# jmg049/Spectrograms

Hardware: AMD Instinct MI355X
Metric: STFT frames/sec (f32, n_fft=1024 hop=256) (higher is better)
Workload: dtype f32

## Files before the change

spectrograms_amd/csrc/kernels_r32x16.hip:

```cpp
#include <type_traits>
#include <utility>

#include "binaural_kind.h"
#include "buffer_ops.h"
#include "fft_inreg.h"
#include "r32x16_layout.h"
#include "sgx_internal.h"

namespace sgx {
namespace {

using namespace inreg;
using namespace r32x16;

typedef int v4i __attribute__((ext_vector_type(4)));
typedef int v2i __attribute__((ext_vector_type(2)));

__device__ __forceinline__ float db_f32(float x) { return __builtin_log2f(x) * 3.01029995663981195f; }

template <int AMP>
__device__ __forceinline__ float amp_f32(float p, float eps) {
    if constexpr (AMP == AMP_MAGNITUDE) return sqrtf(p);
    else if constexpr (AMP == AMP_DB) return db_f32(fmaxf(p, eps));
    else return p;
}
__device__ __forceinline__ float power_of(v2f x) { return __builtin_fmaf(x.x, x.x, x.y * x.y); }

__device__ __forceinline__ unsigned lds_addr(const void *p) { return (unsigned)(size_t)p; }

#ifdef SGX_STAMPS
__device__ unsigned long long g_stamps[32];
#define SGX_STAMP(i)                                                                        \
    do {                                                                                    \
        unsigned long long t_;                                                              \
        __builtin_amdgcn_sched_barrier(0);                                                  \
        asm volatile("s_memtime %0\n\ts_waitcnt lgkmcnt(0)" : "=s"(t_)::"memory");          \
        __builtin_amdgcn_sched_barrier(0);                                                  \
        st_acc[i] += t_ - st_prev;                                                          \
        st_prev = t_;                                                                       \
    } while (0)
#define SGX_STAMP_PARAMS , unsigned long long *st_acc, unsigned long long &st_prev
#define SGX_STAMP_ARGS , st_acc, st_prev
#else
#define SGX_STAMP(i)
#define SGX_STAMP_PARAMS
#define SGX_STAMP_ARGS
#endif

#ifndef SGX_BANDSEG
#define SGX_BANDSEG 0
#endif
#ifndef SGX_BANDTRIP
#define SGX_BANDTRIP 0
#endif
#ifndef SGX_BANDFMA
#define SGX_BANDFMA 0
#endif
#ifndef SGX_BANDPF
#define SGX_BANDPF 0
#endif
#ifndef SGX_ODDHOP
#define SGX_ODDHOP 1
#endif
#ifndef SGX_DMA
#define SGX_DMA 0
#endif
#ifndef SGX_ONEPATH
#define SGX_ONEPATH 1
#endif

template <int OFF>
__device__ __forceinline__ void ds_read64(v2f &d, unsigned addr) {
    asm volatile("ds_read_b64 %0, %1 offset:%2" : "=v"(d) : "v"(addr), "n"(OFF));
}
template <int OFF>
__device__ __forceinline__ void ds_read128(v4f &d, unsigned addr) {
    asm volatile("ds_read_b128 %0, %1 offset:%2" : "=v"(d) : "v"(addr), "n"(OFF));
}
template <int N>
__device__ __forceinline__ void tie8(v2f *d) {
    if constexpr (N >= 0)
        asm volatile("s_waitcnt lgkmcnt(%8)"
                     : "+v"(d[0]), "+v"(d[1]), "+v"(d[2]), "+v"(d[3]), "+v"(d[4]), "+v"(d[5]), "+v"(d[6]), "+v"(d[7])
                     : "n"(N));
    else
        asm volatile("" : "+v"(d[0]), "+v"(d[1]), "+v"(d[2]), "+v"(d[3]), "+v"(d[4]), "+v"(d[5]), "+v"(d[6]), "+v"(d[7]));
}
template <int N>
__device__ __forceinline__ void tie16(v2f (&d)[16]) {
    tie8<N>(&d[0]);
    tie8<-1>(&d[8]);
}
template <bool XSPAD, int N1>
constexpr int col_off() { return N1 * 128 + (XSPAD ? (N1 >> 3) * 128 : 0); }
template <bool XSPAD, int PAR, int... K>
__device__ __forceinline__ void read_cols(v2f (&x)[16], v2f (&w)[16], unsigned xaddr, unsigned waddr, std::integer_sequence<int, K...>) {
    ((ds_read64<col_off<XSPAD, 2 * K + PAR>()>(x[K], xaddr), ds_read64<(2 * K + PAR) * 128>(w[K], waddr)), ...);
}

template <int HOP>
constexpr int p512_off_a(int n1) { return 64 * n1 + (64 * n1 / (8 * HOP)) * 64; }
template <int HOP>
constexpr int p512_off_b(int n1) { return 64 * n1 + 4 * HOP + ((64 * n1 + 4 * HOP) / (8 * HOP)) * 64; }
template <int O0, int O1>
__device__ __forceinline__ void ds_read2x32(v2f &d, unsigned addr) {
    static_assert(O0 >= 0 && O0 < 256 && O1 >= 0 && O1 < 256, "ds_read2_b32: 8-bit dword offsets");
    asm volatile("ds_read2_b32 %0, %1 offset0:%2 offset1:%3" : "=v"(d) : "v"(addr), "n"(O0), "n"(O1));
}
template <int HOP, int PAR, int... K>
__device__ __forceinline__ void read_cols512(v2f (&x)[16], v2f (&w)[16], const unsigned (&base)[8], unsigned waddr, std::integer_sequence<int, K...>) {
    ((ds_read2x32<(p512_off_a<HOP>(2 * K + PAR) - p512_off_a<HOP>((2 * K + PAR) & ~3)) / 4, (p512_off_b<HOP>(2 * K + PAR) - p512_off_a<HOP>((2 * K + PAR) & ~3)) / 4>(
          x[K], base[(2 * K + PAR) >> 2]),
      ds_read64<(2 * K + PAR) * 128>(w[K], waddr)),
     ...);
}

template <int PAR, int... K>
__device__ __forceinline__ void read_cols_odd(v2f (&x)[16], v2f (&w)[16], const unsigned (&base)[4], unsigned waddr, std::integer_sequence<int, K...>) {
    ((ds_read2x32<((2 * K + PAR) & 7) * 32, ((2 * K + PAR) & 7) * 32 + 1>(x[K], base[(2 * K + PAR) >> 3]), ds_read64<(2 * K + PAR) * 128>(w[K], waddr)), ...);
}

template <int PAR, int... K>
__device__ __forceinline__ void read_win(v2f (&w)[16], unsigned waddr, std::integer_sequence<int, K...>) {
    (ds_read64<(2 * K + PAR) * 128>(w[K], waddr), ...);
}

template <int OFF>
__device__ __forceinline__ void dma16_to_lds(__amdgpu_buffer_rsrc_t r, int voff, unsigned lds_base) {
    unsigned keep;
    asm volatile("s_mov_b32 %0, m0\n\ts_mov_b32 m0, %3\n\ts_nop 0\n\tbuffer_load_dwordx4 %1, %2, 0 offen offset:%4 lds\n\ts_mov_b32 m0, %0"
                 : "=&s"(keep)
                 : "v"(voff), "s"(r), "s"(lds_base), "n"(OFF)
                 : "memory");
}
template <bool XSPAD, int R, int ROUNDS>
__device__ __forceinline__ void dma_rounds(__amdgpu_buffer_rsrc_t r, int voff, unsigned xs_base, unsigned wave) {
    if constexpr (R < ROUNDS) {
        const unsigned c0 = R * 256u + wave * 64u;
        dma16_to_lds<0>(r, voff + R * 4096, xs_base + c0 * 16u + (XSPAD ? (c0 >> 6) * 128u : 0u));
        dma_rounds<XSPAD, R + 1, ROUNDS>(r, voff, xs_base, wave);
    }
}

template <bool CONJ>
__device__ __forceinline__ v2f cmul_reg(v2f x, v2f t) {
    const v2f c = x * lo2(t);
    v2f r;
    if constexpr (CONJ) asm("v_pk_fma_f32 %0, %1, %2, %3 op_sel:[1,1,0] op_sel_hi:[0,1,1] neg_hi:[0,1,0]" : "=v"(r) : "v"(x), "v"(t), "v"(c));
    else asm("v_pk_fma_f32 %0, %1, %2, %3 op_sel:[1,1,0] op_sel_hi:[0,1,1] neg_lo:[0,1,0]" : "=v"(r) : "v"(x), "v"(t), "v"(c));
    return r;
}
__device__ __forceinline__ v2f split_tw(v2f D, v2f w) {
    const v2f c = lo2(D) * w;
    v2f r;
    asm("v_pk_fma_f32 %0, %1, %2, %3 op_sel:[1,1,0] op_sel_hi:[1,0,1] neg_lo:[0,1,0]" : "=v"(r) : "v"(D), "v"(w), "v"(c));
    return r;
}

__device__ __forceinline__ void load_tw1(const StftArgs &a, unsigned n2, v2f (&twa)[4], v2f (&twb)[8]) {
    const v2f *t1 = (const v2f *)a.tw1 + n2;
#pragma unroll
    for (int q = 0; q < 4; ++q) twa[q] = t1[16 * 8 * q];
#pragma unroll
    for (int q = 0; q < 8; ++q) twb[q] = t1[16 * q];
}

template <bool P2>
__device__ __forceinline__ void twiddle_store(v2f (&xr)[32], const v2f (&twa)[4], const v2f (&twb)[8], unsigned char *dst) {
#pragma unroll
    for (int k1 = 0; k1 < 32; ++k1) {
        const int qa = k1 >> 3, qb = k1 & 7;
        v2f r = xr[k1];
        if constexpr (P2) {
            if (k1 == 0) r = cmul_reg<true>(r, twa[2]);
        } else {
            if (qb) r = cmulv(r, twb[qb]);
            if (qa) r = cmulv(r, twa[qa]);
        }
#if defined(SGX_ABL_NOEXW)
        asm volatile("" ::"v"(r), "v"(dst));
#elif defined(SGX_ABL_ADDTID)
        asm volatile("ds_write_addtid_b32 %0 offset:%2\n\tds_write_addtid_b32 %1 offset:%3" ::"v"(r.x), "v"(r.y), "n"(k1 * 512), "n"(k1 * 512 + 256) : "memory");
#else
        *(v2f *)(dst + k1 * 128) = r;
#endif
    }
}

__device__ __forceinline__ void read_rows(const unsigned char *exf, unsigned ra, unsigned rb, v2f (&A)[16], v2f (&B)[16]) {
    const v4f *pa = (const v4f *)(exf + ra * 128);
    const v4f *pb = (const v4f *)(exf + rb * 128);
#pragma unroll
    for (int c = 0; c < 8; ++c) {
        const v4f q = pa[c];
        A[2 * c] = (v2f){q.x, q.y};
        A[2 * c + 1] = (v2f){q.z, q.w};
    }
#pragma unroll
    for (int c = 0; c < 8; ++c) {
        const v4f q = pb[c];
        B[2 * c] = (v2f){q.x, q.y};
        B[2 * c + 1] = (v2f){q.z, q.w};
    }
}

struct JobOfs {
    unsigned a1, b1, a2, b2, mid;
};
__device__ __forceinline__ JobOfs job_offsets(unsigned j, unsigned n_frames) {
    const unsigned c1 = j == 0 ? 16u : j, c2 = j == 0 ? 0u : j + 256u;
    return JobOfs{c1 * n_frames, (512u - 224u - c1) * n_frames, c2 * n_frames, (512u - 224u - c2) * n_frames, 256u * n_frames};
}

__device__ __forceinline__ void pass2_twiddle(v2f (&A)[16], v2f (&B)[16], const v2f (&t)[16]) {
#pragma unroll
    for (int n = 1; n < 16; ++n) {
        A[n] = cmul_reg<false>(A[n], t[n]);
        B[n] = cmul_reg<true>(B[n], t[n]);
    }
}

struct PwAddr {
    float *up, *down;
};
template <int MODE, int AMP, bool PWT, bool ROT>
__device__ __forceinline__ void pass2_compute(v2f (&A)[16], v2f (&B)[16], bool j0, float eps, const v4f *tw, __amdgpu_buffer_rsrc_t ro,
                                              unsigned oa1, unsigned ob1, unsigned oa2, unsigned ob2, unsigned omid, unsigned step,
                                              float *pw_c1, float *pw_m1, float *pw_c2, float *pw_m2, float *pw_mid SGX_STAMP_PARAMS) {
    constexpr int R = ROT ? 1 : 0;
    Fft<16, false>::run(A, A);
    Fft<16, false>::run(B, B);
    const v2f a8 = ROT ? B[9] : A[8];
    if (j0) {
        if constexpr (ROT) {
            v2f nA[8], nB[16];
#pragma unroll
            for (int t = 0; t < 8; ++t) nA[t] = B[t + 1];
#pragma unroll
            for (int i = 0; i < 8; ++i) nB[(16 - i) & 15] = A[15 - i];
#pragma unroll
            for (int t = 0; t < 8; ++t) nB[8 - t] = B[(17 - t) & 15];
#pragma unroll
            for (int t = 0; t < 8; ++t) A[8 + t] = nA[t];
#pragma unroll
            for (int i = 0; i < 16; ++i) B[i] = nB[i];
        } else {
            v2f nA[16], nB[8];
#pragma unroll
            for (int i = 0; i < 8; ++i) { nA[i] = B[i]; nA[8 + i] = A[i]; }
            nB[7] = A[0];
#pragma unroll
            for (int t = 1; t < 8; ++t) nB[7 - t] = A[16 - t];
#pragma unroll
            for (int i = 0; i < 16; ++i) A[i] = nA[i];
#pragma unroll
            for (int i = 0; i < 8; ++i) B[i] = nB[i];
        }
        asm volatile("" ::: "memory");
    }
    SGX_STAMP(9);
    constexpr int PSTEP = MODE == OUT_BINAURAL ? 32 * 16 * 2 : PWT ? 32 * 16 : 32;
    auto emit = [&](unsigned voff, unsigned soff, float *pwp, v2f X, bool conj) {
#ifdef SGX_ABL_NOSTORE
        asm volatile("" ::"v"(X), "v"(voff));
        return;
#endif
        if constexpr (MODE == OUT_COMPLEX) {
            const v2f V = conj ? (v2f){X.x, -X.y} : X;
            __builtin_amdgcn_raw_buffer_store_b64(__builtin_bit_cast(v2i, V), ro, (int)voff, (int)soff, 0);
        } else if constexpr (MODE == OUT_MEL) {
#ifdef SGX_ABL_NOPW
            asm volatile("" ::"v"(X), "v"(pwp));
            return;
#endif
            *pwp = AMP == AMP_MAG_IN ? sqrtf(power_of(X)) : power_of(X);
        } else if constexpr (MODE == OUT_BINAURAL) {
            *(v2f *)pwp = conj ? (v2f){X.x, -X.y} : X;
        } else {
            __builtin_amdgcn_raw_buffer_store_b32(__builtin_bit_cast(int, amp_f32<AMP>(power_of(X), eps)), ro, (int)voff, (int)soff, 0);
        }
    };
    auto twi = [&](int i) {
        const v4f q = tw[i >> 1];
        return (i & 1) ? (v2f){q.z, q.w} : (v2f){q.x, q.y};
    };
    auto split = [&](v2f P, v2f Q, v2f w, v2f &X, v2f &Y) {
        const v2f E = pfma(Q, (v2f){1.f, -1.f}, P);
        const v2f D = pfma(Q, (v2f){-1.f, 1.f}, P);
        const v2f T = split_tw(D, w);
        X = E + T;
        Y = E - T;
    };
#pragma unroll
    for (int i = 0; i < 8; ++i) {
        v2f X, Y;
        split(A[i], B[(15 + R - i) & 15], twi(i), X, Y);
        emit(oa1, i * step, pw_c1 + i * PSTEP, X, false);
        emit(ob1, (7 - i) * step, pw_m1 + (7 - i) * PSTEP, Y, true);
    }
#pragma unroll
    for (int t = 0; t < 8; ++t) {
        v2f X, Y;
        split(A[8 + t], B[7 + R - t], twi(8 + t), X, Y);
        emit(oa2, t * step, pw_c2 + t * PSTEP, X, false);
        emit(ob2, (7 - t) * step, pw_m2 + (7 - t) * PSTEP, Y, true);
    }
    if (j0) emit(omid, 0u, pw_mid, a8 * (v2f){2.f, -2.f}, false);
    SGX_STAMP(10);
}

constexpr unsigned kP512Step = 16u * 64u;
template <int MODE, int AMP, bool PACK = false>
__device__ __forceinline__ void pass2_pair512(v2f (&A)[16], v2f (&B)[16], bool j0, float eps, __amdgpu_buffer_rsrc_t ro, unsigned vfull1,
                                              unsigned vhalf1, unsigned vfull2, unsigned vhalf2, unsigned vfullm, unsigned vhalfm, unsigned step,
                                              float *pw1, float *pw2, float *pwm) {
    Fft<16, false>::run(A, A);
    Fft<16, false>::run(B, B);
    const v2f a8 = A[8];
    if (j0) {
        v2f nA[16], nB[8];
#pragma unroll
        for (int i = 0; i < 8; ++i) { nA[i] = B[i]; nA[8 + i] = A[i]; }
        nB[7] = A[0];
#pragma unroll
        for (int t = 1; t < 8; ++t) nB[7 - t] = A[16 - t];
#pragma unroll
        for (int i = 0; i < 16; ++i) A[i] = nA[i];
#pragma unroll
        for (int i = 0; i < 8; ++i) B[i] = nB[i];
        asm volatile("" ::: "memory");
    }
    auto emit = [&](unsigned vfull, unsigned vhalf, int soff, v2f Xa, v2f Xb, bool conj, float *pwp) {
        if constexpr (MODE == OUT_MEL) {
            const float pa = power_of(Xa), pb = power_of(Xb);
            *(v2f *)pwp = AMP == AMP_MAG_IN ? (v2f){sqrtf(pa), sqrtf(pb)} : (v2f){pa, pb};
        } else if constexpr (MODE == OUT_COMPLEX) {
            const float sg = conj ? -1.f : 1.f;
            const v4f V = (v4f){Xa.x, sg * Xa.y, Xb.x, sg * Xb.y};
            if constexpr (PACK) {
                __builtin_amdgcn_raw_buffer_store_b64(__builtin_bit_cast(v2i, (v2f){V.x, V.y}), ro, (int)vfull, soff, 0);
                __builtin_amdgcn_raw_buffer_store_b64(__builtin_bit_cast(v2i, (v2f){V.z, V.w}), ro, (int)vhalf, soff, 0);
            } else {
                __builtin_amdgcn_raw_buffer_store_b128(__builtin_bit_cast(v4i, V), ro, (int)vfull + soff, 0, 0);
                __builtin_amdgcn_raw_buffer_store_b64(__builtin_bit_cast(v2i, (v2f){V.x, V.y}), ro, (int)vhalf, soff, 0);
            }
        } else {
            const v2f V = (v2f){amp_f32<AMP>(power_of(Xa), eps), amp_f32<AMP>(power_of(Xb), eps)};
            if constexpr (PACK) {
                const float va = V.x, vb = V.y;
                __builtin_amdgcn_raw_buffer_store_b32(__builtin_bit_cast(int, va), ro, (int)vfull, soff, 0);
                __builtin_amdgcn_raw_buffer_store_b32(__builtin_bit_cast(int, vb), ro, (int)vhalf, soff, 0);
            } else {
                __builtin_amdgcn_raw_buffer_store_b64(__builtin_bit_cast(v2i, V), ro, (int)vfull, soff, 0);
                __builtin_amdgcn_raw_buffer_store_b32(__builtin_bit_cast(int, V.x), ro, (int)vhalf, soff, 0);
            }
        }
// ... 273 lines not shown
    const unsigned n = lane & 15u, q = lane >> 4;
    const bool mine = mt < a.mfcc_mtiles;
    v4acc acc = {0.f, 0.f, 0.f, 0.f};
    if (mine) {
        const v4f *pa = (const v4f *)(frag + ((size_t)mt * 64u + lane) * RL);
        const v4f *pb = (const v4f *)(mq + (q * 16u + n) * RL);
        v4f wa[STEPS / 4], vb[STEPS / 4];
#pragma unroll
        for (int g = 0; g < STEPS / 4; ++g) { wa[g] = pa[g]; vb[g] = pb[g]; }
#pragma unroll
        for (int g = 0; g < STEPS / 4; ++g) {
            acc = __builtin_amdgcn_mfma_f32_16x16x4f32(wa[g].x, vb[g].x, acc, 0, 0, 0);
            acc = __builtin_amdgcn_mfma_f32_16x16x4f32(wa[g].y, vb[g].y, acc, 0, 0, 0);
            acc = __builtin_amdgcn_mfma_f32_16x16x4f32(wa[g].z, vb[g].z, acc, 0, 0, 0);
            acc = __builtin_amdgcn_mfma_f32_16x16x4f32(wa[g].w, vb[g].w, acc, 0, 0, 0);
        }
    }
    const float *lift = frag + (size_t)a.mfcc_mtiles * 64u * RL;
    constexpr unsigned kDrop = 0x80000000u;
    const unsigned rows = a.n_mfcc - a.mfcc_skip;
    const unsigned obytes = (rows * a.n_frames - f0) * 4u;
    const __amdgpu_buffer_rsrc_t ro = make_rsrc((const float *)a.out + (size_t)b * rows * a.n_frames + f0, obytes);
    const unsigned mtr = mine ? mt : 0u;
#pragma unroll
    for (int r = 0; r < 4; ++r) {
        const unsigned c = 16u * mtr + 4u * q + r;
        const bool ok = mine && c >= a.mfcc_skip && c < a.n_mfcc && n < nf;
        __builtin_amdgcn_raw_buffer_store_b32(__builtin_bit_cast(int, acc[r] * lift[min(c, a.n_mfcc - 1u)]), ro,
                                              (int)(ok ? ((c - a.mfcc_skip) * a.n_frames + n) * 4u : kDrop), 0, 0);
    }
}

__host__ __device__ constexpr unsigned pwt512_index(unsigned k, unsigned f) { return (k >> 1) * 64u + (f >> 1) * 4u + (k & 1u) * 2u + (f & 1u); }
template <int AMP>
__device__ __forceinline__ void mel_tile_sched512(const StftArgs &a, const float *pwT, const unsigned *sched, unsigned b, unsigned f0,
                                                  unsigned nf, float eps, unsigned tid) {
    const unsigned wave = __builtin_amdgcn_readfirstlane(tid >> 6), lane = tid & 63u, slot = lane >> 4, fp = lane & 15u;
    const unsigned obytes = (a.n_out * a.n_frames - f0) * 4u;
    const __amdgpu_buffer_rsrc_t ro = make_rsrc((const float *)a.out + (size_t)b * a.n_out * a.n_frames + f0, obytes);
    constexpr unsigned kDrop = 0x80000000u;
    const unsigned fo0 = 2u * fp < nf ? 8u * fp : kDrop, fo1 = 2u * fp + 1u < nf ? 8u * fp + 4u : kDrop;
    const uint4 *info = (const uint4 *)(sched + kSchedHdr) + wave * 8u + slot;
    uint4 ca = info[0], cb = info[4];
#pragma unroll
    for (unsigned seg = 0; seg < (unsigned)kSchedSegs; ++seg) {
        const uint4 na = info[(seg + 1u) * 32u], nb = info[(seg + 1u) * 32u + 4u];
        const unsigned L = __builtin_amdgcn_readfirstlane(ca.x);
        const v4f *wa = (const v4f *)((const float *)sched + ca.y), *wb = (const v4f *)((const float *)sched + cb.y);
        const v4f *pa = (const v4f *)(pwT + (ca.z >> 1) * 64u) + fp, *pb = (const v4f *)(pwT + (cb.z >> 1) * 64u) + fp;
        v2f acca = {0.0f, 0.0f}, accb = {0.0f, 0.0f};
        for (unsigned t = 0; t < L; t += 4u) {
            const v4f w4a = wa[t >> 2], a0 = pa[(t >> 1) * 16u], a1 = pa[(t >> 1) * 16u + 16u];
            const v4f w4b = wb[t >> 2], b0 = pb[(t >> 1) * 16u], b1 = pb[(t >> 1) * 16u + 16u];
            acca = mul_add_unfused(w4a.x, (v2f){a0.x, a0.y}, acca);
            accb = mul_add_unfused(w4b.x, (v2f){b0.x, b0.y}, accb);
            acca = mul_add_unfused(w4a.y, (v2f){a0.z, a0.w}, acca);
            accb = mul_add_unfused(w4b.y, (v2f){b0.z, b0.w}, accb);
            acca = mul_add_unfused(w4a.z, (v2f){a1.x, a1.y}, acca);
            accb = mul_add_unfused(w4b.z, (v2f){b1.x, b1.y}, accb);
            acca = mul_add_unfused(w4a.w, (v2f){a1.z, a1.w}, acca);
            accb = mul_add_unfused(w4b.w, (v2f){b1.z, b1.w}, accb);
        }
        const bool ha = ca.w != 0xffffffffu, hb = cb.w != 0xffffffffu;
        const unsigned boa = ca.w * a.n_frames * 4u, bob = cb.w * a.n_frames * 4u;
        __builtin_amdgcn_raw_buffer_store_b32(__builtin_bit_cast(int, amp_f32<AMP>(acca.x, eps)), ro, (int)((ha && fo0 != kDrop) ? boa + fo0 : kDrop), 0, 0);
        __builtin_amdgcn_raw_buffer_store_b32(__builtin_bit_cast(int, amp_f32<AMP>(acca.y, eps)), ro, (int)((ha && fo1 != kDrop) ? boa + fo1 : kDrop), 0, 0);
        __builtin_amdgcn_raw_buffer_store_b32(__builtin_bit_cast(int, amp_f32<AMP>(accb.x, eps)), ro, (int)((hb && fo0 != kDrop) ? bob + fo0 : kDrop), 0, 0);
        __builtin_amdgcn_raw_buffer_store_b32(__builtin_bit_cast(int, amp_f32<AMP>(accb.y, eps)), ro, (int)((hb && fo1 != kDrop) ? bob + fo1 : kDrop), 0, 0);
        ca = na;
        cb = nb;
    }
}

template <int KIND>
__device__ __forceinline__ void binaural_tile(const StftArgs &a, const unsigned char *smem_all, unsigned b, unsigned f0, unsigned nf) {
    binaural::KindConst<float> c;
    c.pi = 3.14159265358979323846f;
    c.two_pi = 2.0f * c.pi;
    c.bw = (float)a.bin_bw;
    c.power = a.bin_power;
    c.wrapped = a.bin_wrapped;
    const v2f *L = (const v2f *)smem_all, *R = (const v2f *)(smem_all + kExBytes);
    float *out = (float *)a.out + ((size_t)b * a.bin_count) * a.n_frames + f0;
    for (unsigned i = threadIdx.x; i < a.bin_count * 16u; i += 512u) {
        const unsigned r = i >> 4, f = i & 15u, k = a.bin_start + r;
        const v2f l = L[k * 16u + f], q = R[k * 16u + f];
        const float v = binaural::binaural_value<float, KIND>(l.x, l.y, q.x, q.y, k, c);
        if (f < nf) out[(size_t)r * a.n_frames + f] = v;
    }
}

template <int MODE, int AMP, int ROUNDS, bool WIDE, bool XSPAD, bool PWT, int HOP512 = 0, bool PACK = false, int MSTEPS = 0>
__global__ __launch_bounds__(512, 2) void k_r32x16(StftArgs a, unsigned per_xcd, unsigned total, unsigned slots) {
    constexpr bool MFCC = MSTEPS != 0;
    static_assert(!MFCC || (PWT && AMP == AMP_DB && HOP512 == 0 && !PACK), "fused MFCC epilogue: Mel-dB on the schedule, n_fft 1024, one-signal tiles");
    constexpr bool P512 = HOP512 != 0;
    constexpr bool BIN = MODE == OUT_BINAURAL;
    static_assert(!BIN || (!WIDE && !PWT && !P512 && !PACK && !MFCC), "binaural: one-signal n_fft 1024 tiles, per-half pass 2");
    constexpr unsigned HS = BIN ? 1u : 2u;
    static_assert(!PACK || (ROUNDS == 0 && !WIDE && !XSPAD && (HOP512 == 0 ? (MODE != OUT_MEL || PWT) : MODE != OUT_MEL)),
                  "PACK: direct loads, one-half tiles; n_fft 1024: scheduled band stage, n_fft 512: per-bin outputs");
    constexpr unsigned SS512 = 8u * HOP512;
    static_assert(!P512 || PACK || (HOP512 % 4 == 0 && ROUNDS * 256 * 4 >= 31 * HOP512 + 512), "P512: 16-byte chunks, the whole tile staged");
    static_assert(!WIDE || MODE != OUT_MEL, "wide pass 2 needs a per-bin output");
    static_assert(!PWT || MODE == OUT_MEL, "PWT is a filterbank layout");
    static_assert(!P512 || (!WIDE && !XSPAD && (ROUNDS > 0 || PACK) && (PWT == (MODE == OUT_MEL))), "P512: staged samples (PACK: per-lane loads), scheduled band stage");
    constexpr bool DMA = SGX_DMA != 0 && PWT && ROUNDS > 0 && !P512;
    constexpr unsigned FPT = P512 ? 32u : 16u;
    constexpr unsigned NB = P512 ? 257u : 513u;
    extern __shared__ __attribute__((aligned(16))) unsigned char smem_all[];
    const unsigned half = __builtin_amdgcn_readfirstlane(threadIdx.x >> 8);
    const unsigned tid = threadIdx.x & 255u;
    constexpr bool H256M = HOP512 == 256 && MODE == OUT_MEL && !PACK;
    constexpr unsigned EXB = H256M ? (unsigned)kExBytesH256 : (unsigned)kExBytes, POFF = H256M ? (unsigned)kOutOffH256 : (unsigned)kOutOff;
    unsigned char *smem = smem_all + half * EXB;
    unsigned char *tabs = smem_all + 2 * EXB;
    if (threadIdx.x < 256u) ((v4f *)(tabs + kWinOff))[threadIdx.x] = ((const v4f *)a.window)[threadIdx.x];
    if (threadIdx.x < 256u) {
        const unsigned jj = threadIdx.x >> 4, ii = threadIdx.x & 15u;
        const v4f q = ((const v4f *)a.tw2)[jj * 17u + ii];
        *(v2f *)(tabs + kTw2Off + jj * kTw2Stride + ii * 8u) = (v2f){q.x, q.y};
        *(v2f *)(tabs + kTrOff + jj * 128u + ii * 8u) = ((const v2f *)a.tw1)[(jj == 0u ? 16u : jj) * 16u + ii];
    }
    unsigned *sched = (unsigned *)(tabs + kMelOff);
    if constexpr (PWT)
        for (unsigned i = threadIdx.x; i < a.mel_sched_words; i += 512u) sched[i] = a.mel_sched[i];
    float *mfrag = (float *)(tabs + kMelOff) + ((a.mel_sched_words + 3u) & ~3u);
    if constexpr (MFCC)
        for (unsigned i = threadIdx.x; i < a.mfcc_frag_words; i += 512u) mfrag[i] = ((const float *)a.mfcc_frag)[i];

    const unsigned xcd = blockIdx.x & 7u, slot = blockIdx.x >> 3;
    const unsigned lo = xcd * per_xcd;
    const unsigned hi = min(lo + per_xcd, total);
    unsigned wid = lo + slot * HS + (BIN ? 0u : half);
    unsigned lead = lo + slot * HS;

    const unsigned p1f = tid >> 4, n2 = tid & 15u;
    const unsigned lane = tid & 63u;
    const unsigned wv_ = WIDE ? threadIdx.x >> 6 : tid >> 6;
    const unsigned jq = WIDE ? lane >> 5 : lane >> 4, p2f = WIDE ? lane & 31u : lane & 15u;
    const unsigned j = wv_ + (WIDE ? 8u : 4u) * jq;
    constexpr bool TWP2 = !P512 && MODE != OUT_MEL;
    constexpr bool TRLDS = TWP2 && ROUNDS == 0 && !WIDE;
    const unsigned ra = j == 0 ? (TWP2 ? 16u : 0u) : j, rb = j == 0 ? (TWP2 ? 0u : 16u) : 32u - j;
    const float eps = (float)a.eps;
    constexpr unsigned ES = MODE == OUT_COMPLEX ? 8u : 4u;
    const JobOfs jo = job_offsets(j, a.n_frames);
    const unsigned step = 32u * a.n_frames * ES;
    const v4f *twj = (const v4f *)(tabs + kTw2Off + j * kTw2Stride);
    v2f twa[4], twb[8], tr[16];
    if constexpr (!TWP2) {
        load_tw1(a, n2, twa, twb);
    } else {
        twa[2] = ((const v2f *)a.tw1)[16 * 16 + n2];
        if constexpr (!TRLDS)
#pragma unroll
            for (int q = 0; q < 16; ++q) tr[q] = ((const v2f *)a.tw1)[ra * 16u + q];
    }

    constexpr int NCR = ROUNDS > 0 ? ROUNDS : 1;
    v4f creg[NCR];
    v2f xd[ROUNDS > 0 ? 1 : 32];
    const unsigned chunks = XSPAD ? 1216u : P512 ? (31u * HOP512 + 512u + 3u) >> 2 : (15u * a.hop + 1024u + 3u) >> 2;
    const unsigned hop = XSPAD ? 256u : (P512 && !PACK) ? (unsigned)HOP512 : a.hop;
    const unsigned row_bytes = (unsigned)a.n_samples * 4u;
    auto load_tile = [&](unsigned w) {
        const unsigned b = w / a.tiles, tile = w - b * a.tiles;
        const unsigned f0 = tile * FPT;
        const __amdgpu_buffer_rsrc_t rx = make_rsrc((const float *)(BIN && half ? a.x2 : a.x) + (size_t)b * a.sample_stride, row_bytes);
        const int tile_lo = (int)(f0 * hop) - (int)a.pad;
        const bool interior = tile_lo >= 0 && (unsigned)tile_lo + (FPT - 1u) * hop + (P512 ? 512u : 1024u) <= (unsigned)a.n_samples;
        if constexpr (ROUNDS > 0) {
#ifdef SGX_ABL_NOGLOAD
            for (int r = 0; r < ROUNDS; ++r) creg[r] = (v4f){(float)w, 1.f, 2.f, (float)r};
            return;
#endif
            const int vo = (tile_lo + 4 * (int)tid) * 4;
            if constexpr (DMA) {
                dma_rounds<XSPAD, 0, ROUNDS>(rx, vo, lds_addr(smem), __builtin_amdgcn_readfirstlane(tid >> 6));
                return;
            }
            if (SGX_ONEPATH || interior || P512) {
#pragma unroll
                for (int r = 0; r < ROUNDS; ++r)
                    if (SGX_ONEPATH || XSPAD || P512 || r * 256u + tid < chunks) creg[r] = __builtin_bit_cast(v4f, __builtin_amdgcn_raw_buffer_load_b128(rx, vo + r * 4096, 0, 0));
            } else {
#pragma unroll
                for (int r = 0; r < ROUNDS; ++r) {
                    v4i c;
#pragma unroll
                    for (int e = 0; e < 4; ++e) c[e] = __builtin_amdgcn_raw_buffer_load_b32(rx, vo + r * 4096 + 4 * e, 0, 0);
                    creg[r] = __builtin_bit_cast(v4f, c);
                }
            }
        } else if constexpr (PACK && P512) {
            const __amdgpu_buffer_rsrc_t rall = make_rsrc(a.x, a.x_bytes);
            const unsigned ns = (unsigned)a.n_samples, PP = (a.n_frames + 1u) >> 1;
            const unsigned q = w * 16u + p1f;
            const bool live = q < a.gframes;
            const unsigned bq = live ? q / PP : 0u, pr = q - bq * PP;
            const int sA = (int)(2u * pr * hop) - (int)a.pad + (int)n2, sB = sA + (int)hop;
            const unsigned row = bq * (unsigned)a.sample_stride;
#pragma unroll
            for (int n1 = 0; n1 < 32; ++n1) {
                const int ia = sA + 16 * n1, ib = sB + 16 * n1;
                const int va = __builtin_amdgcn_raw_buffer_load_b32(rall, (live && (unsigned)ia < ns) ? (int)((row + (unsigned)ia) * 4u) : (int)0xfffffff0u, 0, 0);
                const int vb = __builtin_amdgcn_raw_buffer_load_b32(rall, (live && (unsigned)ib < ns) ? (int)((row + (unsigned)ib) * 4u) : (int)0xfffffff0u, 0, 0);
                xd[n1] = (v2f){__builtin_bit_cast(float, va), __builtin_bit_cast(float, vb)};
            }
        } else if constexpr (PACK) {
            const unsigned g = w * 16u + p1f;
            const bool live = g < a.gframes;
            const unsigned bq = live ? g / a.n_frames : 0u, fq = g - bq * a.n_frames;
            const __amdgpu_buffer_rsrc_t rall = make_rsrc(a.x, a.x_bytes);
            const int s0 = (int)(fq * hop) - (int)a.pad + 2 * (int)n2;
            const unsigned rowo = bq * (unsigned)a.sample_stride;
            const unsigned ns = (unsigned)a.n_samples;
#pragma unroll
            for (int n1 = 0; n1 < 32; ++n1) {
                const int sidx = s0 + 32 * n1;
                const bool in0 = live && (unsigned)sidx < ns;
                v2f v = __builtin_bit_cast(v2f, __builtin_amdgcn_raw_buffer_load_b64(rall, in0 ? (int)((rowo + (unsigned)sidx) * 4u) : (int)0xfffffff0u, 0, 0));
                if ((unsigned)(sidx + 1) >= ns) v.y = 0.0f;
                xd[n1] = v;
            }
        } else {
            const int vo = ((int)(p1f * hop) + tile_lo + 2 * (int)n2) * 4;
            if (SGX_ONEPATH || interior) {
#pragma unroll
                for (int n1 = 0; n1 < 32; ++n1) xd[n1] = __builtin_bit_cast(v2f, __builtin_amdgcn_raw_buffer_load_b64(rx, vo + n1 * 128, 0, 0));
#if SGX_ODDHOP
                if (a.hop & 1u) {
                    const float x0 = __builtin_bit_cast(float, __builtin_amdgcn_raw_buffer_load_b32(rx, 0, 0, 0));
                    const int s0 = (int)(p1f * hop) + tile_lo + 2 * (int)n2;
#pragma unroll
                    for (int n1 = 0; n1 < 32; ++n1)
                        if (s0 + 32 * n1 == -1) xd[n1].y = x0;
                }
#endif
            } else {
#pragma unroll
                for (int n1 = 0; n1 < 32; ++n1) {
                    v2i c;
                    c.x = __builtin_amdgcn_raw_buffer_load_b32(rx, vo + n1 * 128, 0, 0);
                    c.y = __builtin_amdgcn_raw_buffer_load_b32(rx, vo + n1 * 128 + 4, 0, 0);
                    xd[n1] = __builtin_bit_cast(v2f, c);
                }
            }
        }
    };

    if (wid >= hi) wid = lead;
    if (lead < hi) load_tile(wid);
    if constexpr (DMA) asm volatile("s_waitcnt vmcnt(0)" ::: "memory");
    __syncthreads();

    const unsigned xaddr = lds_addr(smem) + p1f * hop * 4u + n2 * 8u + (XSPAD ? p1f * 128u : 0u);
    const unsigned waddr = lds_addr(tabs + kWinOff) + n2 * 8u;

#ifdef SGX_SKEW
    if (MODE == OUT_MEL && half == 1u)
        for (unsigned q = 0; q < SGX_SKEW; ++q) __syncthreads();
#endif
#ifndef SGX_STAGGER
#define SGX_STAGGER 4u
#endif
    if constexpr (MODE != OUT_MEL) {
        for (unsigned q = 0; q < (blockIdx.x >> 3) * SGX_STAGGER; ++q) __builtin_amdgcn_s_sleep(1);
        __syncthreads();
    }
#ifdef SGX_PRIO
    if (half == SGX_PRIO - 1u) __builtin_amdgcn_s_setprio(1);
#endif
#ifdef SGX_STAMPS
    unsigned long long st_acc[16] = {0}, st_prev;
    asm volatile("s_memtime %0\n\ts_waitcnt lgkmcnt(0)" : "=s"(st_prev)::"memory");
#endif
    const unsigned mfcc_mt = (((threadIdx.x & 255u) >> 6) + 4u - half) & 3u;
    float *const mfl = (float *)(smem + kOutOff) - 64 * mfcc_row<MFCC ? MSTEPS : 4>();
    unsigned pvb = 0, pvf0 = 0, pvnf = 0;
    static_assert(!MFCC || kOutOff - 256 * mfcc_row<MFCC ? MSTEPS : 4>() >= 22912, "Mel-dB tile above the staged samples");
    while (lead < hi) {
        const unsigned PP = (a.n_frames + 1u) >> 1;
        const unsigned b = PACK ? (P512 ? wid * 16u / PP : wid * 16u / a.n_frames) : wid / a.tiles, tile = wid - b * a.tiles;
        const unsigned f0 = PACK ? wid * 16u - b * a.n_frames : tile * FPT;
        const unsigned nf = PACK ? min(16u, a.gframes - wid * 16u) : min(FPT, a.n_frames - f0);
        v2f xr[32];
        {
            v2f e[16], o[16], we[16], wo[16];
            if constexpr (ROUNDS > 0) {
                if constexpr (DMA) {
                    asm volatile("s_waitcnt vmcnt(%0)" ::"n"(2 * kSchedSegs) : "memory");
                } else {
#pragma unroll
                for (int r = 0; r < ROUNDS; ++r) {
                    const unsigned c = r * 256u + tid;
                    if (SGX_ONEPATH || XSPAD || P512 || c < chunks) *(v4f *)(smem + c * 16u + (XSPAD ? (c >> 6) * 128u : P512 ? (c * 16u / (P512 ? SS512 : 1u)) * 64u : 0u)) = creg[r];
                }
                }
                SGX_STAMP(0);
                __syncthreads();
                SGX_STAMP(1);
                if constexpr (MFCC) mfcc_tile<MFCC ? MSTEPS : 4>(a, mfl, mfrag, mfcc_mt, pvb, pvf0, pvnf, tid & 63u);
                if constexpr (HOP512 == 256) {
                    const float *pa = (const float *)(smem + p1f * (SS512 + 64u) + n2 * 4u);
#pragma unroll
                    for (int k = 0; k < 16; ++k) {
                        e[k] = (v2f){pa[p512_off_a<256>(2 * k) / 4], pa[p512_off_b<256>(2 * k) / 4]};
                        o[k] = (v2f){pa[p512_off_a<256>(2 * k + 1) / 4], pa[p512_off_b<256>(2 * k + 1) / 4]};
                    }
                    read_win<0>(we, waddr, std::make_integer_sequence<int, 16>{});
                    read_win<1>(wo, waddr, std::make_integer_sequence<int, 16>{});
                    tie16<0>(e);
                    tie16<-1>(o);
                    tie16<-1>(we);
                    tie16<-1>(wo);
                } else if constexpr (P512) {
                    unsigned base[8];
#pragma unroll
                    for (int q = 0; q < 8; ++q) base[q] = lds_addr(smem) + p1f * (SS512 + 64u) + n2 * 4u + (unsigned)p512_off_a<P512 ? HOP512 : 128>(4 * q);
                    read_cols512<P512 ? HOP512 : 128, 0>(e, we, base, waddr, std::make_integer_sequence<int, 16>{});
                    read_cols512<P512 ? HOP512 : 128, 1>(o, wo, base, waddr, std::make_integer_sequence<int, 16>{});
                    tie16<15>(e);
                    tie16<-1>(we);
                } else {
                if (SGX_ODDHOP && !XSPAD && (a.hop & 1u)) {
                    const unsigned base[4] = {xaddr, xaddr + 1024u, xaddr + 2048u, xaddr + 3072u};
                    read_cols_odd<0>(e, we, base, waddr, std::make_integer_sequence<int, 16>{});
                    read_cols_odd<1>(o, wo, base, waddr, std::make_integer_sequence<int, 16>{});
                } else {
                read_cols<XSPAD, 0>(e, we, xaddr, waddr, std::make_integer_sequence<int, 16>{});
                read_cols<XSPAD, 1>(o, wo, xaddr, waddr, std::make_integer_sequence<int, 16>{});
                }
                tie16<15>(e);
                tie16<-1>(we);
                }
            } else {
                const v2f *w2 = (const v2f *)(tabs + kWinOff) + n2;
#pragma unroll
                for (int k = 0; k < 16; ++k) {
                    e[k] = xd[2 * k];
                    o[k] = xd[2 * k + 1];
                    we[k] = w2[32 * k];
                    wo[k] = w2[32 * k + 16];
                }
            }
            Fft<16, true>::run(e, we);
            if constexpr (ROUNDS > 0) {
                tie16<0>(o);
                tie16<-1>(wo);
            }
            Fft<16, true>::run(o, wo);
            Comb<32, 0, v2f>::run(xr, e, o);
        }
        SGX_STAMP(2);
        if constexpr (ROUNDS > 0 || MFCC) __syncthreads();
        SGX_STAMP(3);
#ifdef SGX_ABL_ADDTID
        {
            const unsigned m0v = __builtin_amdgcn_readfirstlane(lds_addr(smem) + (tid >> 6) * 16384u);
            asm volatile("s_mov_b32 m0, %0\n\ts_nop 0" ::"s"(m0v) : "memory");
        }
#endif
        twiddle_store<TWP2>(xr, twa, twb, smem + p1f * kFS + n2 * 8);
        SGX_STAMP(4);
        unsigned next = lead + slots * HS + (BIN ? 0u : half);
        if (next >= hi) next -= BIN ? 0u : half;
        if constexpr (!DMA)
            if (lead + slots * HS < hi) load_tile(next);
        SGX_STAMP(5);
        __syncthreads();
        SGX_STAMP(6);
        constexpr bool ALLSTORE = MODE != OUT_MEL;
        unsigned p2b = b, p2ofs, p2ex;
        if constexpr (WIDE) {
            const unsigned w1 = lead + 1u < hi ? lead + 1u : lead;
            const unsigned b0 = lead / a.tiles, f00 = (lead - b0 * a.tiles) * 16u;
            const unsigned b1 = w1 / a.tiles, f01 = (w1 - b1 * a.tiles) * 16u;
            const unsigned nf0 = min(16u, a.n_frames - f00), nf1 = min(16u, a.n_frames - f01);
            const bool second = p2f >= 16u && w1 != lead;
            const unsigned fle = min(p2f & 15u, (second ? nf1 : nf0) - 1u);
            p2ex = (second ? 16u : 0u) + fle;
            p2ofs = (second ? f01 : f00) + fle + ((second && b1 != b0) ? 513u * a.n_frames : 0u);
            p2b = b0;
        } else if constexpr (P512) {
            p2ex = p2f;
            p2ofs = f0 + 2u * p2f;
        } else if constexpr (PACK) {
            const unsigned p2f_eff = ALLSTORE ? min(p2f, nf - 1u) : p2f;
            const unsigned fl = f0 + p2f_eff, bq = fl / a.n_frames;
            p2ex = p2f_eff;
            p2ofs = bq * NB * a.n_frames + (fl - bq * a.n_frames);
        } else {
            const unsigned p2f_eff = ALLSTORE ? min(p2f, nf - 1u) : p2f;
            p2ex = p2f_eff;
            p2ofs = f0 + p2f_eff;
        }
        v2f A[16], B[16];
        read_rows((WIDE ? smem_all : smem) + p2ex * kFS, ra, rb, A, B);
        if constexpr (TRLDS) {
            const v4f *tq = (const v4f *)(tabs + kTrOff + j * 128u);
#pragma unroll
            for (int q = 0; q < 8; ++q) {
                const v4f t2 = tq[q];
                tr[2 * q] = (v2f){t2.x, t2.y};
                tr[2 * q + 1] = (v2f){t2.z, t2.w};
            }
        }
        if constexpr (TWP2) pass2_twiddle(A, B, tr);
        SGX_STAMP(7);
        __syncthreads();
        SGX_STAMP(8);
        if constexpr (DMA)
            if (lead + slots * HS < hi) load_tile(next);
        float *pwf = (float *)(smem + (PWT ? POFF : 0u));
        if constexpr (MODE == OUT_MEL) {
            if constexpr (P512) {
                for (unsigned i = tid; i < 11u * 32u; i += 256u) pwf[pwt512_index(257u + (i >> 5), i & 31u)] = 0.0f;
            } else if constexpr (PWT) {
                if (tid < 176u) pwf[pwt_index(513u + (tid >> 4), tid & 15u)] = 0.0f;
            } else {
                if (tid < 48u) pwf[(tid / 3u) * kPS + 513u + tid % 3u] = 0.0f;
            }
        }
        if constexpr (BIN) {
            const unsigned c1 = j == 0 ? 16u : j, c2 = j == 0 ? 0u : j + 256u;
            auto slot_of = [&](unsigned k) { return (float *)smem + (k * 16u + p2f) * 2u; };
            pass2_compute<MODE, AMP, false, TWP2>(A, B, j == 0, eps, twj, make_rsrc(a.out, 0u), 0u, 0u, 0u, 0u, 0u, 0u, slot_of(c1),
                                            slot_of(512u - 224u - c1), slot_of(c2), slot_of(512u - 224u - c2), slot_of(256u) SGX_STAMP_ARGS);
            __syncthreads();
            binaural_tile<AMP>(a, smem_all, b, f0, nf);
            __syncthreads();
        } else if constexpr (P512 && PACK) {
            constexpr unsigned kDrop = 0x80000000u;
            const __amdgpu_buffer_rsrc_t ro = make_rsrc((unsigned char *)a.out + (size_t)b * NB * a.n_frames * ES, min(17u, a.batch - b) * NB * a.n_frames * ES);
            const unsigned c1 = j == 0 ? 16u : j, r2 = j == 0 ? 0u : 32u - j;
            const unsigned q = wid * 16u + p2f, bq = q / PP, pr = q - bq * PP;
            const unsigned oA = p2f < nf ? ((bq - b) * NB * a.n_frames + 2u * pr) * ES : kDrop;
            const unsigned oB = (p2f < nf && 2u * pr + 1u < a.n_frames) ? oA + ES : kDrop;
            auto at = [&](unsigned base, unsigned row) { return base == kDrop ? kDrop : base + row * a.n_frames * ES; };
            pass2_pair512<MODE, AMP, true>(A, B, j == 0, eps, ro, at(oA, c1), at(oB, c1), at(oA, r2), at(oB, r2), at(oA, 256u), at(oB, 256u), step,
                                           nullptr, nullptr, nullptr);
        } else if constexpr (P512) {
            constexpr unsigned kDrop = 0x80000000u;
            const __amdgpu_buffer_rsrc_t ro = make_rsrc((unsigned char *)a.out + (size_t)b * NB * a.n_frames * ES, NB * a.n_frames * ES);
            const unsigned c1 = j == 0 ? 16u : j, r2 = j == 0 ? 0u : 32u - j;
            const unsigned nv = 2u * p2f + 1u < nf ? 2u : 2u * p2f < nf ? 1u : 0u;
            const unsigned o1 = (c1 * a.n_frames + p2ofs) * ES, o2 = (r2 * a.n_frames + p2ofs) * ES, om = (256u * a.n_frames + p2ofs) * ES;
            float *pws = pwf + 4u * p2f;
            pass2_pair512<MODE, AMP>(A, B, j == 0, eps, ro, nv == 2u ? o1 : kDrop, nv == 1u ? o1 : kDrop, nv == 2u ? o2 : kDrop,
                                     nv == 1u ? o2 : kDrop, nv == 2u ? om : kDrop, nv == 1u ? om : kDrop, step, pws + pwt512_index(c1, 0u),
                                     pws + pwt512_index(r2, 0u), pws + pwt512_index(256u, 0u));
        } else if (ALLSTORE || p2f < nf) {
            const unsigned c1 = j == 0 ? 16u : j, c2 = j == 0 ? 0u : j + 256u;
            const unsigned long long obytes = (unsigned long long)min(PACK ? 17u : 2u, a.batch - p2b) * 513ull * a.n_frames * ES;
            const __amdgpu_buffer_rsrc_t ro = make_rsrc((unsigned char *)a.out + (size_t)p2b * 513u * a.n_frames * ES, (unsigned)obytes);
            {
                auto slot_of = [&](unsigned k) { return pwf + (PWT ? pwt_index(k, p2f) : p2f * kPS + k); };
                pass2_compute<MODE, AMP, PWT, TWP2>(A, B, j == 0, eps, twj, ro, (jo.a1 + p2ofs) * ES, (jo.b1 + p2ofs) * ES, (jo.a2 + p2ofs) * ES,
                                                     (jo.b2 + p2ofs) * ES, (jo.mid + p2ofs) * ES, step, slot_of(c1), slot_of(512u - 224u - c1),
                                                     slot_of(c2), slot_of(512u - 224u - c2), slot_of(256u) SGX_STAMP_ARGS);
            }
        }
        if constexpr (MODE == OUT_MEL) {
            __syncthreads();
            SGX_STAMP(11);
#ifdef SGX_ABL_NOMEL
            if (a.n_mels == 12345u)
#endif
            if constexpr (P512) mel_tile_sched512<AMP>(a, pwf, sched, b, f0, nf, eps, tid);
            else if constexpr (MFCC) {
                mel_tile_sched<AMP, false, mfcc_row<MFCC ? MSTEPS : 4>()>(a, pwf, sched, b, f0, nf, eps, tid, mfl SGX_STAMP_ARGS);
                if constexpr (ROUNDS > 0) {
                    pvb = b; pvf0 = f0; pvnf = nf;
                } else {
                    __syncthreads();
                    mfcc_tile<MFCC ? MSTEPS : 4>(a, mfl, mfrag, mfcc_mt, b, f0, nf, tid & 63u);
                }
            }
            else if constexpr (PWT) mel_tile_sched<AMP, PACK>(a, pwf, sched, b, f0, nf, eps, tid, nullptr SGX_STAMP_ARGS);
            else if (a.mm_frag) map_tile_mfma<AMP>(a, pwf, b, f0, nf, eps, tid, 2u * half);
            else mel_tile_csr<AMP>(a, pwf, b, f0, nf, eps, tid, 256u);
            if constexpr (!PWT) __syncthreads();
        }
        SGX_STAMP(14);
        wid = next;
        lead += slots * HS;
#ifdef SGX_STAMPS
        st_acc[15] += 1;
#endif
    }
    if constexpr (MFCC && ROUNDS > 0) {
        __syncthreads();
        mfcc_tile<MFCC ? MSTEPS : 4>(a, mfl, mfrag, mfcc_mt, pvb, pvf0, pvnf, tid & 63u);
    }
#ifdef SGX_SKEW
    if (MODE == OUT_MEL && half == 0u)
        for (unsigned q = 0; q < SGX_SKEW; ++q) __syncthreads();
#endif
#ifdef SGX_STAMPS
    if ((threadIdx.x & 63u) == 0) {
        for (int q = 0; q < 16; ++q) atomicAdd(&g_stamps[q], st_acc[q]);
        atomicAdd(&g_stamps[16], 1ull);
    }
#endif
}

static bool want_pack(const StftArgs &a, bool mel, bool pwt) {
    if (a.mfcc_frag) return false;
    const bool p512 = a.n_fft == 512u;
    const bool unlisted512 = p512 && !(a.hop == 64u || a.hop == 128u || a.hop == 160u || a.hop == 256u);
    if ((a.n_fft != 1024u && !p512) || (a.batch < 2u && !unlisted512) || (mel && (!pwt || p512)) || (a.hop & 1u)) return false;
    const unsigned long long slots = (unsigned long long)a.tiles * a.ft, g = (unsigned long long)a.batch * a.n_frames;
    const unsigned long long used = p512 ? 2ull * ((a.n_frames + 1ull) / 2ull) : a.n_frames;
    if ((slots - used) * 4ull < slots && !unlisted512) return false;
    if (g >= 0x7fffffffull || (unsigned long long)a.batch * a.sample_stride * 4ull >= 0xfffffff0ull) return false;
    return (a.ft + 1ull) * (a.n_fft / 2u + 1ull) * a.n_frames * 8ull < 0x7fffffffull;
}

template <int MODE, int AMP>
hipError_t launch_variant(const StftArgs &a0, hipStream_t s) {
    StftArgs a = a0;
    const bool pack = want_pack(a, MODE == OUT_MEL, MODE == OUT_MEL && a.mel_sched != nullptr);
    const bool pack512 = pack && a.n_fft == 512u;
    a.gframes = pack512 ? a.batch * ((a.n_frames + 1u) / 2u) : a.batch * a.n_frames;
    a.x_bytes = pack ? (unsigned)((unsigned long long)a.batch * a.sample_stride * 4ull) : 0u;
    const unsigned total = pack ? (a.gframes + 15u) / 16u : a.tiles * a.batch;
    const unsigned per_xcd = (total + 7) / 8;
    const unsigned chunks = (15u * a.hop + 1024u + 3u) >> 2;
    const unsigned pairs = (per_xcd + 1) / 2;
#ifndef SGX_SLOTS
#define SGX_SLOTS 0u
#endif
    const unsigned cu_slots = SGX_SLOTS ? SGX_SLOTS : std::max(1u, device_cu_count() / 8u);
    const unsigned nslots = pairs < cu_slots ? pairs : cu_slots;
    const bool pwt = MODE == OUT_MEL && a.mel_sched != nullptr;
    auto go = [&](auto kernel, unsigned lds = (unsigned)kLdsBytes) -> hipError_t {
        hipError_t e = set_max_dynamic_lds((const void *)kernel, 163840);
        if (e != hipSuccess) return e;
        hipLaunchKernelGGL(kernel, dim3(nslots * 8), dim3(512), lds, s, a, per_xcd, total, nslots);
        return hipGetLastError();
    };
    constexpr bool W = MODE != OUT_MEL;
    if constexpr (MODE != OUT_MEL)
        if (pack && a.n_fft == 512u) return go(k_r32x16<MODE, AMP, 0, false, false, false, 128, true>);
    if (pack) {
        if (MODE == OUT_MEL) note_bank_stage("r32x16_sched_packed");
        return go(k_r32x16<MODE, AMP, 0, false, false, MODE == OUT_MEL, 0, true>);
    }
    if constexpr (MODE == OUT_MEL) {
        if (pwt) {
            if (a.n_fft == 512u) {
                note_bank_stage("r32x16_sched512");
                if (a.hop == 64u) return go(k_r32x16<MODE, AMP, 3, false, false, true, 64>);
                if (a.hop == 128u) return go(k_r32x16<MODE, AMP, 5, false, false, true, 128>);
                if (a.hop == 160u) return go(k_r32x16<MODE, AMP, 6, false, false, true, 160>);
                if (a.hop == 256u)
                    return go(k_r32x16<MODE, AMP, 9, false, false, true, 256>, 2u * kExBytesH256 + kMelOff + ((a.mel_sched_words * 4u + 15u) & ~15u) + 64u);
                return hipErrorInvalidConfiguration;
            }
            if constexpr (AMP == AMP_DB) {
                if (a.mfcc_frag && a.n_fft == 1024u) {
                    const unsigned lds = (unsigned)kLdsBytes - (unsigned)kMelMaxWords * 4u + ((a.mel_sched_words + 3u) & ~3u) * 4u + a.mfcc_frag_words * 4u + 64u;
                    if (lds > 163840u) return hipErrorInvalidConfiguration;
                    note_bank_stage("r32x16_sched_mfcc");
                    const unsigned ldsz = lds < (unsigned)kLdsBytes ? (unsigned)kLdsBytes : lds;
                    auto mf = [&](auto steps) -> hipError_t {
                        constexpr int S = decltype(steps)::value;
                        if (a.hop == 256u) return go(k_r32x16<MODE, AMP, 5, false, true, true, 0, false, S>, ldsz);
                        if (chunks <= 5u * 256u) return go(k_r32x16<MODE, AMP, 5, false, false, true, 0, false, S>, ldsz);
                        return go(k_r32x16<MODE, AMP, 0, false, false, true, 0, false, S>, ldsz);
                    };
                    if (a.mfcc_steps == 12u) return mf(std::integral_constant<int, 12>{});
                    if (a.mfcc_steps == 16u) return mf(std::integral_constant<int, 16>{});
                    if (a.mfcc_steps == 20u) return mf(std::integral_constant<int, 20>{});
                    if (a.mfcc_steps == 24u) return mf(std::integral_constant<int, 24>{});
                    return hipErrorInvalidConfiguration;
                }
            }
            note_bank_stage("r32x16_sched");
            if (a.hop == 256u) return go(k_r32x16<MODE, AMP, 5, false, true, true>);
            if (chunks <= 5u * 256u) return go(k_r32x16<MODE, AMP, 5, false, false, true>);
            return go(k_r32x16<MODE, AMP, 0, false, false, true>);
        }
    }
    if constexpr (MODE != OUT_MEL) {
        if (a.n_fft == 512u) {
            if (a.hop == 64u) return go(k_r32x16<MODE, AMP, 3, false, false, false, 64>);
            if (a.hop == 128u) return go(k_r32x16<MODE, AMP, 5, false, false, false, 128>);
            if (a.hop == 160u) return go(k_r32x16<MODE, AMP, 6, false, false, false, 160>);
            if (a.hop == 256u) return go(k_r32x16<MODE, AMP, 9, false, false, false, 256>);
            return hipErrorInvalidConfiguration;
        }
    }
    if (a.n_fft != 1024u) return hipErrorInvalidConfiguration;
    if (MODE == OUT_MEL) note_bank_stage(a.mm_frag ? "r32x16_mfma" : "r32x16_csr");
    if (a.hop == 256u) return go(k_r32x16<MODE, AMP, 5, W, true, false>);
    if (chunks <= 5u * 256u) return go(k_r32x16<MODE, AMP, 5, W, false, false>);
    return go(k_r32x16<MODE, AMP, 0, W, false, false>);
}

template <int KIND>
hipError_t launch_binaural(const StftArgs &a, hipStream_t s) {
    const unsigned total = a.tiles * a.batch;
    const unsigned per_xcd = (total + 7) / 8;
    const unsigned chunks = (15u * a.hop + 1024u + 3u) >> 2;
    const unsigned cu_slots = SGX_SLOTS ? SGX_SLOTS : std::max(1u, device_cu_count() / 8u);
    const unsigned nslots = per_xcd < cu_slots ? per_xcd : cu_slots;
    auto go = [&](auto kernel) -> hipError_t {
        hipError_t e = set_max_dynamic_lds((const void *)kernel, 163840);
        if (e != hipSuccess) return e;
        hipLaunchKernelGGL(kernel, dim3(nslots * 8), dim3(512), (unsigned)kLdsBytes, s, a, per_xcd, total, nslots);
        return hipGetLastError();
    };
    if (a.hop == 256u) return go(k_r32x16<OUT_BINAURAL, KIND, 5, false, true, false>);
    if (chunks <= 5u * 256u) return go(k_r32x16<OUT_BINAURAL, KIND, 5, false, false, false>);
    return go(k_r32x16<OUT_BINAURAL, KIND, 0, false, false, false>);
}

}

#ifdef SGX_STAMPS
extern "C" int sgx_debug_read_stamps(unsigned long long *out, int reset) {
    if (hipMemcpyFromSymbol(out, HIP_SYMBOL(g_stamps), sizeof(g_stamps)) != hipSuccess) return 1;
    if (reset) {
        unsigned long long z[32] = {0};
        if (hipMemcpyToSymbol(HIP_SYMBOL(g_stamps), z, sizeof(z)) != hipSuccess) return 1;
    }
    return 0;
}
#endif

bool plan_geometry_r32x16_f32(StftArgs &a) {
    if (a.n_fft == 512 && a.hop == 256 && a.out_mode == OUT_MEL && a.mel_sched_words > (unsigned)kMelMaxWordsH256) return false;
    if (a.n_fft == 512 && a.out_mode == OUT_MEL && a.mel_sched_words == 0) return false;
    if (a.n_fft == 512 && (a.hop == 64 || a.hop == 128 || a.hop == 160 || a.hop == 256)) {
        if (a.n_samples >= (1ull << 29) || (unsigned long long)a.n_frames * 257ull * 8ull >= 0x7fffffffull) return false;
        a.ft = 32;
        return true;
    }
    if (a.n_fft == 512) {
        if (a.out_mode == OUT_MEL || (a.hop & 1u) || a.hop > 512u) return false;
        if (a.n_samples >= (1ull << 29) || (unsigned long long)a.batch * a.n_frames >= 0x7fffffffull ||
// ... 41 lines not shown
```

Measured before the change: 1.470 billion.

## Double-buffer global sample loads two tiles ahead in wide round path

Adds a second register buffer for staged input samples so the wide, register-round path prefetches the tile two iterations ahead instead of one. The main loop becomes a lambda called alternately with the two buffers, which hides more global-load latency behind the FFT passes. The twa[2] twiddle is now reloaded from the LDS table each round instead of held in registers, and the row offsets are pinned in VGPRs. The extra buffer raises register pressure and may reduce occupancy.

```diff
diff --git a/spectrograms_amd/csrc/kernels_r32x16.hip b/spectrograms_amd/csrc/kernels_r32x16.hip
--- a/spectrograms_amd/csrc/kernels_r32x16.hip
+++ b/spectrograms_amd/csrc/kernels_r32x16.hip
@@ -65,6 +65,12 @@
 #ifndef SGX_DMA
 #define SGX_DMA 0
 #endif
+#ifndef SGX_DEEP
+#define SGX_DEEP 1
+#endif
+#ifndef SGX_DEEP_ISSUE
+#define SGX_DEEP_ISSUE 0
+#endif
 #ifndef SGX_ONEPATH
 #define SGX_ONEPATH 1
 #endif
@@ -187,9 +193,9 @@
     }
 }
 
-__device__ __forceinline__ void read_rows(const unsigned char *exf, unsigned ra, unsigned rb, v2f (&A)[16], v2f (&B)[16]) {
-    const v4f *pa = (const v4f *)(exf + ra * 128);
-    const v4f *pb = (const v4f *)(exf + rb * 128);
+__device__ __forceinline__ void read_rows_at(const unsigned char *exf, unsigned oa, unsigned ob, v2f (&A)[16], v2f (&B)[16]) {
+    const v4f *pa = (const v4f *)(exf + oa);
+    const v4f *pb = (const v4f *)(exf + ob);
 #pragma unroll
     for (int c = 0; c < 8; ++c) {
         const v4f q = pa[c];
@@ -202,6 +208,9 @@
         B[2 * c] = (v2f){q.x, q.y};
         B[2 * c + 1] = (v2f){q.z, q.w};
     }
+}
+__device__ __forceinline__ void read_rows(const unsigned char *exf, unsigned ra, unsigned rb, v2f (&A)[16], v2f (&B)[16]) {
+    read_rows_at(exf, ra * 128u, rb * 128u, A, B);
 }
 
 struct JobOfs {
@@ -781,19 +790,22 @@
     if constexpr (!TWP2) {
         load_tw1(a, n2, twa, twb);
     } else {
-        twa[2] = ((const v2f *)a.tw1)[16 * 16 + n2];
+        if constexpr (!(SGX_DEEP != 0 && ROUNDS > 0 && WIDE)) twa[2] = ((const v2f *)a.tw1)[16 * 16 + n2];
         if constexpr (!TRLDS)
 #pragma unroll
             for (int q = 0; q < 16; ++q) tr[q] = ((const v2f *)a.tw1)[ra * 16u + q];
     }
 
     constexpr int NCR = ROUNDS > 0 ? ROUNDS : 1;
-    v4f creg[NCR];
+    constexpr bool DEEP = SGX_DEEP != 0 && ROUNDS > 0 && WIDE;
+    v4f creg[NCR], creg2[DEEP ? NCR : 1];
+    unsigned rowa = ra * 128u, rowb = rb * 128u;
+    if constexpr (DEEP) asm volatile("" : "+v"(rowa), "+v"(rowb));
     v2f xd[ROUNDS > 0 ? 1 : 32];
     const unsigned chunks = XSPAD ? 1216u : P512 ? (31u * HOP512 + 512u + 3u) >> 2 : (15u * a.hop + 1024u + 3u) >> 2;
     const unsigned hop = XSPAD ? 256u : (P512 && !PACK) ? (unsigned)HOP512 : a.hop;
     const unsigned row_bytes = (unsigned)a.n_samples * 4u;
-    auto load_tile = [&](unsigned w) {
+    auto load_tile = [&](unsigned w, v4f (&cr)[NCR]) {
         const unsigned b = w / a.tiles, tile = w - b * a.tiles;
         const unsigned f0 = tile * FPT;
         const __amdgpu_buffer_rsrc_t rx = make_rsrc((const float *)(BIN && half ? a.x2 : a.x) + (size_t)b * a.sample_stride, row_bytes);
@@ -801,7 +813,7 @@
         const bool interior = tile_lo >= 0 && (unsigned)tile_lo + (FPT - 1u) * hop + (P512 ? 512u : 1024u) <= (unsigned)a.n_samples;
         if constexpr (ROUNDS > 0) {
 #ifdef SGX_ABL_NOGLOAD
-            for (int r = 0; r < ROUNDS; ++r) creg[r] = (v4f){(float)w, 1.f, 2.f, (float)r};
+            for (int r = 0; r < ROUNDS; ++r) cr[r] = (v4f){(float)w, 1.f, 2.f, (float)r};
             return;
 #endif
             const int vo = (tile_lo + 4 * (int)tid) * 4;
@@ -812,14 +824,14 @@
             if (SGX_ONEPATH || interior || P512) {
 #pragma unroll
                 for (int r = 0; r < ROUNDS; ++r)
-                    if (SGX_ONEPATH || XSPAD || P512 || r * 256u + tid < chunks) creg[r] = __builtin_bit_cast(v4f, __builtin_amdgcn_raw_buffer_load_b128(rx, vo + r * 4096, 0, 0));
+                    if (SGX_ONEPATH || XSPAD || P512 || r * 256u + tid < chunks) cr[r] = __builtin_bit_cast(v4f, __builtin_amdgcn_raw_buffer_load_b128(rx, vo + r * 4096, 0, 0));
             } else {
 #pragma unroll
                 for (int r = 0; r < ROUNDS; ++r) {
                     v4i c;
 #pragma unroll
                     for (int e = 0; e < 4; ++e) c[e] = __builtin_amdgcn_raw_buffer_load_b32(rx, vo + r * 4096 + 4 * e, 0, 0);
-                    creg[r] = __builtin_bit_cast(v4f, c);
+                    cr[r] = __builtin_bit_cast(v4f, c);
                 }
             }
         } else if constexpr (PACK && P512) {
@@ -880,7 +892,12 @@
     };
 
     if (wid >= hi) wid = lead;
-    if (lead < hi) load_tile(wid);
+    if (lead < hi) load_tile(wid, creg);
+    if constexpr (DEEP) {
+        unsigned w2 = lead + slots * HS + half;
+        if (w2 >= hi) w2 -= half;
+        if (lead + slots * HS < hi) load_tile(w2, creg2);
+    }
     if constexpr (DMA) asm volatile("s_waitcnt vmcnt(0)" ::: "memory");
     __syncthreads();
 
@@ -909,7 +926,7 @@
     float *const mfl = (float *)(smem + kOutOff) - 64 * mfcc_row<MFCC ? MSTEPS : 4>();
     unsigned pvb = 0, pvf0 = 0, pvnf = 0;
     static_assert(!MFCC || kOutOff - 256 * mfcc_row<MFCC ? MSTEPS : 4>() >= 22912, "Mel-dB tile above the staged samples");
-    while (lead < hi) {
+    auto round = [&](v4f (&cr)[NCR]) __attribute__((always_inline)) {
         const unsigned PP = (a.n_frames + 1u) >> 1;
         const unsigned b = PACK ? (P512 ? wid * 16u / PP : wid * 16u / a.n_frames) : wid / a.tiles, tile = wid - b * a.tiles;
         const unsigned f0 = PACK ? wid * 16u - b * a.n_frames : tile * FPT;
@@ -924,7 +941,7 @@
 #pragma unroll
                 for (int r = 0; r < ROUNDS; ++r) {
                     const unsigned c = r * 256u + tid;
-                    if (SGX_ONEPATH || XSPAD || P512 || c < chunks) *(v4f *)(smem + c * 16u + (XSPAD ? (c >> 6) * 128u : P512 ? (c * 16u / (P512 ? SS512 : 1u)) * 64u : 0u)) = creg[r];
+                    if (SGX_ONEPATH || XSPAD || P512 || c < chunks) *(v4f *)(smem + c * 16u + (XSPAD ? (c >> 6) * 128u : P512 ? (c * 16u / (P512 ? SS512 : 1u)) * 64u : 0u)) = cr[r];
                 }
                 }
                 SGX_STAMP(0);
@@ -991,15 +1008,24 @@
             asm volatile("s_mov_b32 m0, %0\n\ts_nop 0" ::"s"(m0v) : "memory");
         }
 #endif
+        if constexpr (DEEP) twa[2] = *(const v2f *)(tabs + kTrOff + n2 * 8u);
         twiddle_store<TWP2>(xr, twa, twb, smem + p1f * kFS + n2 * 8);
         SGX_STAMP(4);
         unsigned next = lead + slots * HS + (BIN ? 0u : half);
         if (next >= hi) next -= BIN ? 0u : half;
-        if constexpr (!DMA)
-            if (lead + slots * HS < hi) load_tile(next);
+        unsigned next2 = lead + 2u * slots * HS + half;
+        if (next2 >= hi) next2 -= half;
+        auto load_ahead = [&]() {
+            if (lead + 2u * slots * HS < hi) load_tile(next2, cr);
+        };
+        if constexpr (DEEP) {
+            if constexpr (SGX_DEEP_ISSUE == 0) load_ahead();
+        } else if constexpr (!DMA)
+            if (lead + slots * HS < hi) load_tile(next, cr);
         SGX_STAMP(5);
         __syncthreads();
         SGX_STAMP(6);
+        if constexpr (DEEP && SGX_DEEP_ISSUE == 1) load_ahead();
         constexpr bool ALLSTORE = MODE != OUT_MEL;
         unsigned p2b = b, p2ofs, p2ex;
         if constexpr (WIDE) {
@@ -1026,7 +1052,8 @@
             p2ofs = f0 + p2f_eff;
         }
         v2f A[16], B[16];
-        read_rows((WIDE ? smem_all : smem) + p2ex * kFS, ra, rb, A, B);
+        if constexpr (DEEP) read_rows_at(smem_all + p2ex * kFS, rowa, rowb, A, B);
+        else read_rows((WIDE ? smem_all : smem) + p2ex * kFS, ra, rb, A, B);
         if constexpr (TRLDS) {
             const v4f *tq = (const v4f *)(tabs + kTrOff + j * 128u);
 #pragma unroll
@@ -1040,8 +1067,9 @@
         SGX_STAMP(7);
         __syncthreads();
         SGX_STAMP(8);
+        if constexpr (DEEP && SGX_DEEP_ISSUE == 2) load_ahead();
         if constexpr (DMA)
-            if (lead + slots * HS < hi) load_tile(next);
+            if (lead + slots * HS < hi) load_tile(next, cr);
         float *pwf = (float *)(smem + (PWT ? POFF : 0u));
         if constexpr (MODE == OUT_MEL) {
             if constexpr (P512) {
@@ -1118,6 +1146,15 @@
 #ifdef SGX_STAMPS
         st_acc[15] += 1;
 #endif
+    };
+    if constexpr (DEEP) {
+        while (lead + slots * HS < hi) {
+            round(creg);
+            round(creg2);
+        }
+        if (lead < hi) round(creg);
+    } else {
+        while (lead < hi) round(creg);
     }
     if constexpr (MFCC && ROUNDS > 0) {
         __syncthreads();
```

Result: slower. 1.407 billion (-4.2%).
